# idonahum/photoVerse

Hardware: AMD Instinct MI355X
Metric: denoising steps/sec at 512x512 bs=16, 50-step loop (2 UNet fwd + CFG + DPM-Solver++ step per step) (higher is better)
Workload: dtype f16; 1 GPU; configs[1] shape timed over 96 steps instead of 50: SD-v1.5 UNet + PhotoVerse processors, 96-step loop, bs=16/GPU, 512x512 (64x64 latents), P=1, guidance 7.5, fp16; per_gpu_batch=16, global_batch=16, latent=64, parallelism=dp1 (batch-sharded, 1 all_gather), hip_graph=True, graph_branches=2

## Files before the change

### photoverse_amd/csrc/pv_attn.hip

```cpp
#include "pv_common.h"
#include <type_traits>

#ifndef PV_ATTN8_DEFAULT
#define PV_ATTN8_DEFAULT 497
#endif
#ifndef PV_ATTN8_FENCE_LOOP
#define PV_ATTN8_FENCE_LOOP 1
#endif
#ifndef PV_ATTN8_MAX3
#define PV_ATTN8_MAX3 1
#endif
#ifndef PV_ATTN8_RECOMPUTE
#define PV_ATTN8_RECOMPUTE 1
#endif
#ifndef PV_ATTN8_REDO_HINT
#define PV_ATTN8_REDO_HINT 0
#endif
#ifndef PV_ATTN8_LOOP_PAD
#define PV_ATTN8_LOOP_PAD 4
#endif
#ifndef PV_ATTN_LAZY_UP
#define PV_ATTN_LAZY_UP 8.f
#endif
#ifndef PV_ATTN_ABLATE
#define PV_ATTN_ABLATE 0
#endif

#ifdef PV_ATTN8_STAMPS
__device__ unsigned long long pv_attn8_stamps[3 * 8 * 8];
extern "C" int pv_attn8_read_stamps(unsigned long long* out) { return (int)hipMemcpyFromSymbol(out, HIP_SYMBOL(pv_attn8_stamps), sizeof(pv_attn8_stamps)); }
#define A8_NOW() __builtin_amdgcn_s_memtime()
#endif

namespace {

template <int D>
struct ACfg {
    static constexpr int DK = (D + 31) / 32 * 32;
    static constexpr int KSTEPS = DK / 32;
    static constexpr int DVF = (D + 15) / 16;
    static constexpr bool KSWZ = DK == 64;
    static constexpr int KS = KSWZ ? DK : DK + 8;
    static constexpr int KCH = KS / 8;
    __device__ static __forceinline__ int koff(int row, int chunk) {
        return KSWZ ? row * KS + ((chunk ^ (row & 7)) << 3) : row * KS + (chunk << 3);
    }
    static constexpr int vs_dwords() {
        int v = DVF * 8;
        while ((v & 63) != 8 && (v & 63) != 24 && (v & 63) != 40 && (v & 63) != 56) v += 4;
        return v;
    }
    static constexpr int VS = vs_dwords() * 2;
    static constexpr int CH = D / 8;
};

__device__ __forceinline__ half8_t zero8() { return half8_t{0, 0, 0, 0, 0, 0, 0, 0}; }

__device__ __forceinline__ half8_t vt_frag(const half_t* sV, int VS, int key0, int dv0, int fr, int fq) {
    const half_t* a = sV + (key0 + fq * 4 + (fr >> 2)) * VS + dv0 + (fr & 3) * 4;
    const fp16x4_t t1 = __builtin_amdgcn_ds_read_tr16_b64_v4f16((__attribute__((address_space(3))) fp16x4_t*)(a));
    const fp16x4_t t2 = __builtin_amdgcn_ds_read_tr16_b64_v4f16((__attribute__((address_space(3))) fp16x4_t*)(a + 16 * VS));
    half8_t r;
#pragma unroll
    for (int j = 0; j < 4; ++j) {
        r[j] = (half_t)t1[j];
        r[j + 4] = (half_t)t2[j];
    }
    return r;
}

template <int D>
constexpr int attn_min_waves() { return 1; }

template <int D, int NQ, bool DMA>
__global__ __launch_bounds__(256, attn_min_waves<D>()) void attn_kernel(const pv_attn_params p) {
    using C = ACfg<D>;
    static_assert(!DMA || (C::KSWZ && C::VS == 48 && D == 40), "the DMA staging is laid out for d = 40 (128-B swizzled K rows, 96-B V rows)");
    constexpr int KB = 64;
    constexpr int NCHUNK = KB * C::CH;
    constexpr int KPT = (NCHUNK + 255) / 256;
#ifdef PV_ATTN_NO_ONES
    constexpr bool ONES = false;
#else
    constexpr bool ONES = (D % 16) != 0;
#endif
    constexpr bool DBUF = false;
    constexpr int STAGE = KB * (C::KS + C::VS);
    extern __shared__ __attribute__((aligned(16))) char smem[];
    half_t* sbase = reinterpret_cast<half_t*>(smem);

    const int tid = threadIdx.x, lane = tid & 63, wave = pv_wave_id();
    const int fr = lane & 15, fq = lane >> 4;
    constexpr int QW = 64 * NQ;
    const int nqt = (p.nq + QW - 1) / QW;
    const int rid = pv_xcd_remap((int)blockIdx.x, (int)gridDim.x);
    const int qt = rid % nqt, h = (rid / nqt) % p.heads, b = rid / (nqt * p.heads);
    const half_t* Q = reinterpret_cast<const half_t*>(p.q) + (size_t)b * p.nq * p.ldq + h * D;
    const half_t* Kg = reinterpret_cast<const half_t*>(p.k) + (size_t)b * p.nk * p.ldk + h * D;
    const half_t* Vg = reinterpret_cast<const half_t*>(p.v) + (size_t)b * p.nk * p.ldv + h * D;

    for (int st = 0; st < (DMA ? 4 : DBUF ? 2 : 1); ++st) {
        half_t* sK = sbase + st * STAGE;
        half_t* sV = sK + KB * C::KS;
        constexpr int NPC = C::KCH - C::CH, NPV = (C::VS - D) / 8;
        for (int i = tid; i < KB * NPC; i += 256) {
            const int r = i / NPC, c = i - r * NPC;
            *reinterpret_cast<half8_t*>(sK + C::koff(r, C::CH + c)) = zero8();
        }
        for (int i = tid; i < KB * NPV; i += 256) {
            const int r = i / NPV, c = i - r * NPV;
            half8_t v = zero8();
            if (ONES && c == 0) v[0] = (half_t)1.0f;
            *reinterpret_cast<half8_t*>(sV + r * C::VS + D + c * 8) = v;
        }
    }

    const float qscale = rsqrtf((float)D) * 1.4426950408889634f;
    half8_t qf[NQ][C::KSTEPS];
    int qrow[NQ];
#pragma unroll
    for (int qi = 0; qi < NQ; ++qi) {
        qrow[qi] = qt * QW + (wave * NQ + qi) * 16 + fr;
        const int rc = min(qrow[qi], p.nq - 1);
#pragma unroll
        for (int ks = 0; ks < C::KSTEPS; ++ks) {
            const int c = ks * 4 + fq;
            qf[qi][ks] = c < C::CH ? *reinterpret_cast<const half8_t*>(Q + (size_t)rc * p.ldq + c * 8) : zero8();
#pragma unroll
            for (int j = 0; j < 8; ++j) qf[qi][ks][j] = (half_t)((float)qf[qi][ks][j] * qscale);
        }
    }

    half8_t kreg[KPT], vreg[KPT];
    auto gload = [&](int t) {
#pragma unroll
        for (int i = 0; i < KPT; ++i) {
            const int idx = tid + i * 256;
            const int key = idx / C::CH, c = idx - key * C::CH;
            const int gk = t * KB + key;
            if (idx < NCHUNK && gk < p.nk) {
                kreg[i] = *reinterpret_cast<const half8_t*>(Kg + (size_t)gk * p.ldk + c * 8);
                vreg[i] = *reinterpret_cast<const half8_t*>(Vg + (size_t)gk * p.ldv + c * 8);
            } else {
                kreg[i] = zero8();
                vreg[i] = zero8();
            }
        }
    };
    auto swrite = [&](int st) {
        half_t* sK = sbase + st * STAGE;
        half_t* sV = sK + KB * C::KS;
#pragma unroll
        for (int i = 0; i < KPT; ++i) {
            const int idx = tid + i * 256;
            const int key = idx / C::CH, c = idx - key * C::CH;
            if (idx < NCHUNK) {
                *reinterpret_cast<half8_t*>(sK + C::koff(key, c)) = kreg[i];
                *reinterpret_cast<half8_t*>(sV + key * C::VS + c * 8) = vreg[i];
            }
        }
    };

    float4_t o[C::DVF][NQ];
#pragma unroll
    for (int f = 0; f < C::DVF; ++f)
#pragma unroll
        for (int qi = 0; qi < NQ; ++qi) o[f][qi] = float4_t{0.f, 0.f, 0.f, 0.f};
    float m_run[NQ], l_run[NQ];
#pragma unroll
    for (int qi = 0; qi < NQ; ++qi) m_run[qi] = l_run[qi] = 0.f;

    auto tile = [&](int t, int st, const bool MASKED, const bool FIRST) {
        const half_t* sK = sbase + st * STAGE;
        const half_t* sV = sK + KB * C::KS;
        float4_t s[4][NQ];
#pragma unroll
        for (int qi = 0; qi < NQ; ++qi) {
            const float init = FIRST ? 0.f : -m_run[qi];
#pragma unroll
            for (int kb = 0; kb < 4; ++kb) s[kb][qi] = float4_t{init, init, init, init};
        }
#pragma unroll
        for (int ks = 0; ks < C::KSTEPS; ++ks)
#pragma unroll
            for (int kb = 0; kb < 4; ++kb) {
                const half8_t a = *reinterpret_cast<const half8_t*>(sK + C::koff(kb * 16 + fr, ks * 4 + fq));
#pragma unroll
#if PV_ATTN_ABLATE == 2
                asm volatile("" ::"v"(a));
#else
                for (int qi = 0; qi < NQ; ++qi) s[kb][qi] = __builtin_amdgcn_mfma_f32_16x16x32_f16(a, qf[qi][ks], s[kb][qi], 0, 0, 0);
#endif
            }
        half8_t pb[2][NQ];
#pragma unroll
        for (int qi = 0; qi < NQ; ++qi) {
            if (MASKED) {
#pragma unroll
                for (int kb = 0; kb < 4; ++kb)
#pragma unroll
                    for (int r = 0; r < 4; ++r) {
                        const int key = t * KB + kb * 16 + fq * 4 + r;
                        if (key >= p.nk || (p.causal && key > qrow[qi])) s[kb][qi][r] = -INFINITY;
                    }
            }
            float mx = -INFINITY;
#pragma unroll
            for (int kb = 0; kb < 4; ++kb)
#pragma unroll
                for (int r = 0; r < 4; ++r) mx = fmaxf(mx, s[kb][qi][r]);
            mx = pv_quad_max(mx);
            float d = 0.f;
            if (FIRST || __any(mx > PV_ATTN_LAZY_UP)) {
                d = FIRST ? (mx == -INFINITY ? 0.f : mx) : fmaxf(mx, 0.f);
                const float alpha = FIRST ? 0.f : PV_EXP2(-d);
                m_run[qi] += d;
                if (!ONES) l_run[qi] *= alpha;
#pragma unroll
                for (int f = 0; f < C::DVF; ++f) o[f][qi] *= alpha;
#pragma unroll
                for (int kb = 0; kb < 4; ++kb)
#pragma unroll
                    for (int r = 0; r < 4; ++r) s[kb][qi][r] -= d;
            }
            float rs = 0.f;
#pragma unroll
            for (int kb = 0; kb < 4; ++kb)
#pragma unroll
                for (int r = 0; r < 4; ++r) {
#if PV_ATTN_ABLATE == 1
                    const float e = s[kb][qi][r];
#else
                    const float e = PV_EXP2(s[kb][qi][r]);
#endif
                    if (!ONES) rs += e;
                    s[kb][qi][r] = e;
                }
            if (!ONES) l_run[qi] += rs;
#pragma unroll
            for (int s2 = 0; s2 < 2; ++s2)
#pragma unroll
                for (int r = 0; r < 4; ++r) {
                    pb[s2][qi][r] = (half_t)s[2 * s2][qi][r];
                    pb[s2][qi][r + 4] = (half_t)s[2 * s2 + 1][qi][r];
                }
        }
#pragma unroll
        for (int s2 = 0; s2 < 2; ++s2)
#pragma unroll
            for (int f = 0; f < C::DVF; ++f) {
                const half8_t a = vt_frag(sV, C::VS, s2 * 32, f * 16, fr, fq);
#if PV_ATTN_ABLATE == 3
                asm volatile("" ::"v"(a), "v"(pb[s2][0]), "v"(pb[s2][1]));
#else
#pragma unroll
                for (int qi = 0; qi < NQ; ++qi) o[f][qi] = __builtin_amdgcn_mfma_f32_16x16x32_f16(a, pb[s2][qi], o[f][qi], 0, 0, 0);
#endif
            }
    };

    int ntiles = (p.nk + KB - 1) / KB;
    if (p.causal) ntiles = min(ntiles, (min(qt * QW + QW - 1, p.nq - 1)) / KB + 1);
    if constexpr (DMA) {
        const __amdgpu_buffer_rsrc_t rk = __builtin_amdgcn_make_buffer_rsrc(const_cast<half_t*>(Kg), 0, ((p.nk - 1) * p.ldk + D) * 2, 0x00020000);
        const __amdgpu_buffer_rsrc_t rv = __builtin_amdgcn_make_buffer_rsrc(const_cast<half_t*>(Vg), 0, ((p.nk - 1) * p.ldv + D) * 2, 0x00020000);
        constexpr unsigned OOB = 0x80000000u;
        unsigned koff[2], voff[2];
        bool vlive[2];
#pragma unroll
        for (int i = 0; i < 2; ++i) {
            const int r = 8 * (wave + 4 * i) + (lane >> 3), c = (lane & 7) ^ (lane >> 3);
            koff[i] = c < C::CH ? (unsigned)(r * p.ldk * 2 + c * 16) : OOB;
            const int q = 64 * (wave + 4 * i) + lane, vr = q / 6, vc = q - vr * 6;
            voff[i] = (unsigned)(vr * p.ldv * 2 + vc * 16);
            vlive[i] = vc < C::CH;
        }
        auto issue_tile = [&](int t) {
            char* sK = reinterpret_cast<char*>(sbase + (t & 3) * STAGE);
            char* sV = sK + KB * C::KS * 2;
            const int sk = t * KB * p.ldk * 2, sv = t * KB * p.ldv * 2;
#pragma unroll
            for (int i = 0; i < 2; ++i) __builtin_amdgcn_raw_ptr_buffer_load_lds(rk, PV_LDS_PTR(sK + (wave + 4 * i) * 1024), 16, (int)koff[i], sk, 0, 0);
            if (vlive[0]) __builtin_amdgcn_raw_ptr_buffer_load_lds(rv, PV_LDS_PTR(sV + wave * 1024), 16, (int)voff[0], sv, 0, 0);
            if (wave < 2) {
                if (vlive[1]) __builtin_amdgcn_raw_ptr_buffer_load_lds(rv, PV_LDS_PTR(sV + (wave + 4) * 1024), 16, (int)voff[1], sv, 0, 0);
            }
        };
        __syncthreads();
        issue_tile(0);
        if (ntiles > 1) issue_tile(1);
        for (int t = 0; t < ntiles; ++t) {
            if ((t & 1) == 0) {
                asm volatile("s_waitcnt vmcnt(0)" ::: "memory");
                asm volatile("s_waitcnt lgkmcnt(0)" ::: "memory");
                __builtin_amdgcn_s_barrier();
                asm volatile("" ::: "memory");
                if (t + 2 < ntiles) issue_tile(t + 2);
                if (t + 3 < ntiles) issue_tile(t + 3);
            }
            const bool need_mask = p.causal || (t + 1) * KB > p.nk;
            tile(t, t & 3, need_mask, t == 0);
        }
    } else {
    gload(0);
    if (DBUF) {
        swrite(0);
        __syncthreads();
    }
    for (int t = 0; t < ntiles; ++t) {
        const int st = DBUF ? (t & 1) : 0;
        if (!DBUF) {
            __syncthreads();
            swrite(0);
            __syncthreads();
        }
        if (t + 1 < ntiles) gload(t + 1);
        const bool need_mask = p.causal || (t + 1) * KB > p.nk;
        tile(t, st, need_mask, t == 0);
        if (DBUF) {
            if (t + 1 < ntiles) swrite(st ^ 1);
            __syncthreads();
        }
    }
    }

    half_t* O = reinterpret_cast<half_t*>(p.out) + (size_t)b * p.nq * p.ldo + h * D;
#pragma unroll
    for (int qi = 0; qi < NQ; ++qi) {
        float l;
        if (ONES) {
            l = __shfl(o[D / 16][qi][D % 4], fr + 16 * ((D % 16) / 4), 64);
        } else {
            l = pv_quad_sum(l_run[qi]);
        }
        const float inv = 1.0f / l;
        if (p.lse != nullptr && fq == 0 && qrow[qi] < p.nq) p.lse[((size_t)b * p.heads + h) * p.nq + qrow[qi]] = m_run[qi] + __log2f(l);
        if (qrow[qi] < p.nq) {
#pragma unroll
            for (int f = 0; f < C::DVF; ++f) {
                const int dv = f * 16 + fq * 4;
                if (dv < D) {
                    half4_t ov;
#pragma unroll
                    for (int r = 0; r < 4; ++r) ov[r] = (half_t)(o[f][qi][r] * inv);
                    *reinterpret_cast<half4_t*>(O + (size_t)qrow[qi] * p.ldo + dv) = ov;
                }
            }
        }
    }
}

template <int VAR>
__global__ __launch_bounds__(512, 2) void attn8_kernel(const pv_attn_params p) {
    constexpr int D = 40, NQ = 4, KB = 64;
    using C = ACfg<D>;
    constexpr bool STAGGER = (VAR & 1) != 0, PRIO = (VAR & 2) != 0, PCHECK = (VAR & 32) != 0, JOINT = (VAR & 4) != 0 || PCHECK, LAZY = (VAR & 8) != 0 || PCHECK;
    constexpr bool SEGPRIO = (VAR & 16) != 0, PREF = (VAR & 64) != 0, K48 = (VAR & 128) != 0;
    constexpr bool DMA_IN_VEC = PREF && (VAR & 256) != 0;
    constexpr float UP = LAZY ? 8.f : 0.f;
    constexpr int STAGE = KB * (C::KS + C::VS);
    extern __shared__ __attribute__((aligned(16))) char smem[];
    half_t* sbase = reinterpret_cast<half_t*>(smem);

    const int tid = threadIdx.x, lane = tid & 63, wave = pv_wave_id();
    const int fr = lane & 15, fq = lane >> 4;
    const bool late = STAGGER && wave >= 4;
    constexpr int QW = 64 * NQ * 2;
    const int nqt = (p.nq + QW - 1) / QW;
    const int rid = pv_xcd_remap((int)blockIdx.x, (int)gridDim.x);
    const int qt = rid % nqt, h = (rid / nqt) % p.heads, b = rid / (nqt * p.heads);
    const half_t* Q = reinterpret_cast<const half_t*>(p.q) + (size_t)b * p.nq * p.ldq + h * D;
    const half_t* Kg = reinterpret_cast<const half_t*>(p.k) + (size_t)b * p.nk * p.ldk + h * D;
    const half_t* Vg = reinterpret_cast<const half_t*>(p.v) + (size_t)b * p.nk * p.ldv + h * D;

    for (int st = 0; st < 4; ++st) {
        half_t* sK = sbase + st * STAGE;
        half_t* sV = sK + KB * C::KS;
        constexpr int NPC = C::KCH - C::CH, NPV = (C::VS - D) / 8;
        for (int i = tid; i < KB * NPC; i += 512) {
            const int r = i / NPC, c = i - r * NPC;
            *reinterpret_cast<half8_t*>(sK + C::koff(r, C::CH + c)) = zero8();
        }
        for (int i = tid; i < KB * NPV; i += 512) {
            const int r = i / NPV, c = i - r * NPV;
// ... 499 lines not shown
                    *reinterpret_cast<half4_t*>(O + (size_t)qrow[qi] * p.ldo + dv) = ov;
                }
            }
        }
    }
    }
}

enum AttnKind { ATTN8 = 0, ATTN40_4_DMA, ATTN40_2_DMA, ATTN_4, ATTN_2 };
struct AttnChoice {
    AttnKind kind;
    int var8;
    long wgs;
};
#define PV_A8_VARIANTS(X) X(0) X(1) X(9) X(13) X(33) X(49) X(73) X(201) X(225) X(241) X(481) X(497)
constexpr bool attn8_variant_built(int v) {
#define PV_A8_TEST(V) if (v == V) return true;
    PV_A8_VARIANTS(PV_A8_TEST)
#undef PV_A8_TEST
    return false;
}
static_assert(attn8_variant_built(PV_ATTN8_DEFAULT), "the default variant must be an instantiated one");

template <int D>
AttnChoice choose_attn(const pv_attn_params& p) {
    static const int nq_env = getenv("PV_ATTN_NQ") ? atoi(getenv("PV_ATTN_NQ")) : 0;
    const long wg256 = (long)((p.nq + 255) / 256) * p.heads * p.batch, wg128 = (long)((p.nq + 127) / 128) * p.heads * p.batch;
    const bool four = D == 40 && (nq_env ? nq_env == 4 : wg256 >= 1024);
    if constexpr (D == 40) {
        static const bool no_dma = getenv("PV_ATTN_NO_DMA") != nullptr;
        if (!no_dma && (size_t)p.nk * (size_t)(p.ldk > p.ldv ? p.ldk : p.ldv) * 2 < (1ull << 31)) {
            const char* env8 = getenv("PV_ATTN8");
            const char* env8min = getenv("PV_ATTN8_MIN");
            const int var8 = env8 ? atoi(env8) : PV_ATTN8_DEFAULT;
            const long wg512 = (long)((p.nq + 511) / 512) * p.heads * p.batch;
            if (attn8_variant_built(var8) && !p.causal && wg512 >= (env8min ? atol(env8min) : 256)) return {ATTN8, var8, wg512};
            return four ? AttnChoice{ATTN40_4_DMA, 0, wg256} : AttnChoice{ATTN40_2_DMA, 0, wg128};
        }
    }
    return four ? AttnChoice{ATTN_4, 0, wg256} : AttnChoice{ATTN_2, 0, wg128};
}

template <int D>
int launch_attn(const pv_attn_params& p, hipStream_t s) {
    using C = ACfg<D>;
    constexpr int smem1 = 64 * (C::KS + C::VS) * 2;
    const AttnChoice ch = choose_attn<D>(p);
    if constexpr (D == 40) {
        constexpr int smem3 = 4 * smem1;
        if (ch.kind == ATTN8) {
            void (*kern)(const pv_attn_params) = nullptr;
            switch (ch.var8) {
#define PV_A8_CASE(V) case V: kern = attn8_kernel<V>; break;
                PV_A8_VARIANTS(PV_A8_CASE)
#undef PV_A8_CASE
                default: return (int)hipErrorInvalidValue;
            }
            static bool attr8_set[64][512] = {};
            int dev8 = 0;
            (void)hipGetDevice(&dev8);
            if (!attr8_set[dev8 & 63][ch.var8 & 511]) {
                const hipError_t e = hipFuncSetAttribute(reinterpret_cast<const void*>(kern), hipFuncAttributeMaxDynamicSharedMemorySize, smem3);
                if (e != hipSuccess) return (int)e;
                attr8_set[dev8 & 63][ch.var8 & 511] = true;
            }
            hipLaunchKernelGGL(kern, dim3((unsigned)ch.wgs), dim3(512), smem3, s, p);
            return PV_CHECK_LAUNCH();
        }
        if (ch.kind == ATTN40_4_DMA || ch.kind == ATTN40_2_DMA) {
            static bool attr_set_dev[64] = {};
            int dev_id = 0;
            (void)hipGetDevice(&dev_id);
            if (!attr_set_dev[dev_id & 63]) {
                hipError_t e = hipFuncSetAttribute(reinterpret_cast<const void*>(attn_kernel<40, 4, true>), hipFuncAttributeMaxDynamicSharedMemorySize, smem3);
                if (e == hipSuccess) e = hipFuncSetAttribute(reinterpret_cast<const void*>(attn_kernel<40, 2, true>), hipFuncAttributeMaxDynamicSharedMemorySize, smem3);
                if (e != hipSuccess) return (int)e;
                attr_set_dev[dev_id & 63] = true;
            }
            if (ch.kind == ATTN40_4_DMA) hipLaunchKernelGGL((attn_kernel<40, 4, true>), dim3((unsigned)ch.wgs), dim3(256), smem3, s, p);
            else hipLaunchKernelGGL((attn_kernel<40, 2, true>), dim3((unsigned)ch.wgs), dim3(256), smem3, s, p);
            return PV_CHECK_LAUNCH();
        }
    }
    if (ch.kind == ATTN_4) hipLaunchKernelGGL((attn_kernel<D, D == 40 ? 4 : 2, false>), dim3((unsigned)ch.wgs), dim3(256), smem1, s, p);
    else hipLaunchKernelGGL((attn_kernel<D, 2, false>), dim3((unsigned)ch.wgs), dim3(256), smem1, s, p);
    return PV_CHECK_LAUNCH();
}

template <int D>
int attn_info(const pv_attn_params& p, char* name, int name_len, int64_t* workgroups) {
    const AttnChoice ch = choose_attn<D>(p);
    int n;
    switch (ch.kind) {
        case ATTN8: n = snprintf(name, (size_t)name_len, "attn8_kernel<%d>", ch.var8); break;
        case ATTN40_4_DMA: n = snprintf(name, (size_t)name_len, "attn_kernel<40, 4, true>"); break;
        case ATTN40_2_DMA: n = snprintf(name, (size_t)name_len, "attn_kernel<40, 2, true>"); break;
        case ATTN_4: n = snprintf(name, (size_t)name_len, "attn_kernel<%d, 4, false>", D); break;
        default: n = snprintf(name, (size_t)name_len, "attn_kernel<%d, 2, false>", D); break;
    }
    if (n < 0 || n >= name_len) return (int)hipErrorInvalidValue;
    if (workgroups) *workgroups = ch.wgs;
    return 0;
}

template <int D>
int launch_xattn(const pv_xattn_params& p, hipStream_t s) {
    using C = ACfg<D>;
    constexpr int smem = XKEYS * (C::KS + C::VS) * 2;
    static bool attr_set_dev[64] = {};
    int dev_id = 0;
    (void)hipGetDevice(&dev_id);
    bool& attr_set = attr_set_dev[dev_id & 63];
    if (smem > 48 * 1024 && !attr_set) {
        hipError_t e = hipFuncSetAttribute(reinterpret_cast<const void*>(xattn_kernel<D, false>), hipFuncAttributeMaxDynamicSharedMemorySize, smem);
        if (e == hipSuccess) e = hipFuncSetAttribute(reinterpret_cast<const void*>(xattn_kernel<D, true>), hipFuncAttributeMaxDynamicSharedMemorySize, smem);
        if (e != hipSuccess) return (int)e;
        attr_set = true;
    }
    const int nqt = (p.nq + 127) / 128;
    const long wgs = (long)nqt * p.heads * p.batch;
    int qt_per_wg = (int)(wgs / 1024);
    qt_per_wg = qt_per_wg < 1 ? 1 : (qt_per_wg > 4 ? 4 : qt_per_wg);
    const int nqg = (nqt + qt_per_wg - 1) / qt_per_wg;
    if (qt_per_wg > 1) hipLaunchKernelGGL((xattn_kernel<D, true>), dim3(nqg * p.heads * p.batch), dim3(256), smem, s, p, qt_per_wg);
    else hipLaunchKernelGGL((xattn_kernel<D, false>), dim3(nqg * p.heads * p.batch), dim3(256), smem, s, p, 1);
    return PV_CHECK_LAUNCH();
}

}

extern "C" int pv_attention(const pv_attn_params* p, void* stream) {
    if (!p->q || !p->k || !p->v || !p->out || p->batch <= 0 || p->heads <= 0 || p->nq <= 0 || p->nk <= 0 || (p->ldq % 8) ||
        (p->ldk % 8) || (p->ldv % 8) || (p->ldo % 4))
        return (int)hipErrorInvalidValue;
    hipStream_t s = (hipStream_t)stream;
    switch (p->d) {
        case 40: return launch_attn<40>(*p, s);
        case 64: return launch_attn<64>(*p, s);
        case 80: return launch_attn<80>(*p, s);
        case 160: return launch_attn<160>(*p, s);
        default: return (int)hipErrorInvalidValue;
    }
}

extern "C" int pv_attention_kernel_info(const pv_attn_params* p, char* name, int32_t name_len, int64_t* workgroups) {
    if (!p || !name || name_len <= 0 || p->batch <= 0 || p->heads <= 0 || p->nq <= 0 || p->nk <= 0) return (int)hipErrorInvalidValue;
    switch (p->d) {
        case 40: return attn_info<40>(*p, name, name_len, workgroups);
        case 64: return attn_info<64>(*p, name, name_len, workgroups);
        case 80: return attn_info<80>(*p, name, name_len, workgroups);
        case 160: return attn_info<160>(*p, name, name_len, workgroups);
        default: return (int)hipErrorInvalidValue;
    }
}

extern "C" int pv_cross_attention(const pv_xattn_params* p, void* stream) {
    if (!p->q || !p->kt || !p->vt || !p->kip || !p->vip || !p->out || p->batch <= 0 || p->heads <= 0 || p->nq <= 0 || p->nt <= 0 ||
        p->nt > IP0 || p->nip <= 0 || p->nip > XKEYS - IP0 || (p->ldq % 8) || (p->ldkt % 8) || (p->ldvt % 8) || (p->ldkip % 8) ||
        (p->ldvip % 8) || (p->ldo % 4))
        return (int)hipErrorInvalidValue;
    hipStream_t s = (hipStream_t)stream;
    switch (p->d) {
        case 40: return launch_xattn<40>(*p, s);
        case 80: return launch_xattn<80>(*p, s);
        case 160: return launch_xattn<160>(*p, s);
        default: return (int)hipErrorInvalidValue;
// ... 3 lines not shown
```

### photoverse_amd/build.py

```python
from __future__ import annotations

import concurrent.futures as cf
import os
import shutil
import subprocess
import sys

HERE = os.path.dirname(os.path.abspath(__file__))
CSRC = os.path.join(HERE, "csrc")
LIBDIR = os.path.join(HERE, "lib")
LIB = os.path.join(LIBDIR, "libphotoverse_hip.so")
SOURCES = ["pv_gemm.hip", "pv_convbig.hip", "pv_norm.hip", "pv_attn.hip", "pv_misc.hip", "pv_xfused.hip", "pv_xq.hip", "pv_rowgemm.hip", "pv_backward.hip", "pv_train.hip", "pv_attnbwd.hip"]
FLAGS = ["--offload-arch=gfx950", "-O3", "-std=c++17", "-fPIC"]
EXTRA_FLAGS = {"pv_attn.hip": ["-mllvm", "-amdgpu-mfma-vgpr-form", "-fno-honor-nans"],
               "pv_xfused.hip": ["-mllvm", "-amdgpu-mfma-vgpr-form", "-fno-honor-nans",
                                 "-mllvm", "-pragma-unroll-threshold=4000000"],

               "pv_xq.hip": ["-mllvm", "-amdgpu-mfma-vgpr-form", "-fno-honor-nans"],
               "pv_rowgemm.hip": ["-mllvm", "-amdgpu-mfma-vgpr-form"],
               "pv_train.hip": ["-mllvm", "-amdgpu-mfma-vgpr-form", "-fno-honor-nans"],
               "pv_attnbwd.hip": ["-mllvm", "-amdgpu-mfma-vgpr-form", "-fno-honor-nans"]}


def _hipcc() -> str:
    exe = shutil.which("hipcc") or "/opt/rocm/bin/hipcc"
    if not os.path.exists(exe):
        raise RuntimeError("hipcc not found: the HIP extension cannot be built")
    return exe


def _stale(out: str, deps) -> bool:
    if not os.path.exists(out):
        return True
    t = os.path.getmtime(out)
    return any(os.path.getmtime(d) > t for d in deps)


def build_lib(force: bool = False, verbose: bool = True) -> str:
    os.makedirs(LIBDIR, exist_ok=True)
    hipcc = _hipcc()
    headers = [os.path.join(CSRC, "pv_common.h"), os.path.join(CSRC, "pv_gemm_dev.h"), os.path.join(os.path.dirname(HERE), "include", "photoverse_hip.h"), __file__]
    objs, jobs = [], []
    for src in SOURCES:
        s = os.path.join(CSRC, src)
        o = os.path.join(LIBDIR, src.replace(".hip", ".o"))
        objs.append(o)
        if force or _stale(o, [s] + headers):
            jobs.append([hipcc, *FLAGS, *EXTRA_FLAGS.get(src, []), "-c", s, "-o", o])
    if jobs:
        with cf.ThreadPoolExecutor(max_workers=4) as ex:
            for cmd, res in zip(jobs, ex.map(lambda c: subprocess.run(c, capture_output=True, text=True), jobs)):
                if res.returncode != 0:
                    raise RuntimeError("hipcc failed: %s\n%s" % (" ".join(cmd), res.stderr))
                if verbose:
                    print("[photoverse_amd.build] compiled", os.path.basename(cmd[-3]))
    if jobs or force or _stale(LIB, objs):
        res = subprocess.run([hipcc, "--offload-arch=gfx950", "-shared", "-fPIC", "-o", LIB, *objs], capture_output=True, text=True)
        if res.returncode != 0:
            raise RuntimeError("link failed:\n" + res.stderr)
        if verbose:
            print("[photoverse_amd.build] linked", LIB)
    return LIB


if __name__ == "__main__":
    build_lib(force="--force" in sys.argv)
```

### photoverse_amd/csrc/pv_gemm.hip

```cpp
#include "pv_gemm_dev.h"

namespace {

constexpr int BK = 64;
constexpr int ROW_BYTES = BK * 2;

template <int NF, int MIV = 4>
struct TileCfg {
    static constexpr int MI = MIV;
    static constexpr int BM = 2 * MI * 16;
    static constexpr int BN = NF * 32;
    static constexpr int NWAVES = 4;
    static constexpr int THREADS = NWAVES * 64;
    static constexpr int A_PER_WAVE = BM / 8 / NWAVES;
    static constexpr int STAGES = 2;
    static constexpr int A_BYTES = BM * ROW_BYTES;
    static constexpr int B_BYTES = BN * ROW_BYTES;
    static constexpr int STAGE_BYTES = A_BYTES + B_BYTES;
    static constexpr int SMEM_BYTES = STAGES * STAGE_BYTES;
    static constexpr int B_PIECES = NF * 4;
    static constexpr int B_PER_WAVE = (B_PIECES + NWAVES - 1) / NWAVES;
};

__device__ __forceinline__ float epi_act(float x, int act) {
// ... 452 lines not shown

template <int NF>
int choose_tpw(const pv_gemm_params_dev& p) {
    static const int tpw_env = getenv("PV_GEMM_TPW") ? atoi(getenv("PV_GEMM_TPW")) : 0;
    if (p.taps != 1 || (p.splitk > 1 && p.splitk_ws)) return 1;
    const int tiles_n = p.N / (NF * 32), nk = (p.c0 + p.c1) / BK;
    const long nblk = (long)((p.M + 127) / 128) * tiles_n;
    if (tpw_env > 0) return tiles_n % tpw_env == 0 ? tpw_env : 1;
    for (int c = 8; c >= 2; --c)
        if (tiles_n % c == 0 && nk <= 5 && nblk / c >= 1024) return c;
    return 1;
}

template <int NF, bool CONV, bool GEGLU>
int dispatch(const pv_gemm_params_dev& p, hipStream_t stream) {
    if constexpr (!CONV && GEGLU) {
        const int tpw = choose_tpw<NF>(p);
        if (tpw > 1) return launch<NF, false, true, false, true>(p, stream, tpw);
    }
    if constexpr (!GEGLU) {
        if (p.colstats && !(p.splitk > 1 && p.splitk_ws)) return launch<NF, CONV, false, true>(p, stream);
    }
    if constexpr (!CONV && !GEGLU) {
        static const int mi2_env = getenv("PV_GEMM_MI2") ? atoi(getenv("PV_GEMM_MI2")) : 512;
        const long tiles128 = (long)((p.M + 127) / 128) * (p.N / (NF * 32));
        if (!(p.splitk > 1 && p.splitk_ws) && tiles128 < mi2_env) return launch<NF, false, false, false, false, 2>(p, stream);
    }
    return launch<NF, CONV, GEGLU>(p, stream);
}

}

int pv_gemm_splitk_reduce_launch(const pv_gemm_params_dev& p, int splits, hipStream_t stream) {
    hipLaunchKernelGGL(splitk_reduce_kernel, dim3((unsigned)((p.N + 63) / 64), (unsigned)((p.M + 63) / 64)), dim3(256), 0, stream, p, splits);
    return PV_CHECK_LAUNCH();
}

thread_local pv_launch_probe* pv_gemm_probe = nullptr;

extern "C" int pv_gemm_conv(const pv_gemm_params* pp, void* stream_);

extern "C" int pv_gemm_conv_kernel_info(const pv_gemm_params* pp, char* name, int32_t name_len, int64_t* workgroups) {
    if (!pp || !name || name_len <= 0) return (int)hipErrorInvalidValue;
    pv_launch_probe probe;
    probe.name[0] = 0;
    probe.wgs = 0;
    pv_gemm_probe = &probe;
    const int rc = pv_gemm_conv(pp, nullptr);
    pv_gemm_probe = nullptr;
    if (rc != 0) return rc;
    if ((int)strlen(probe.name) >= name_len) return (int)hipErrorInvalidValue;
    strcpy(name, probe.name);
    if (workgroups) *workgroups = probe.wgs;
    return 0;
}

extern "C" int pv_gemm_conv(const pv_gemm_params* pp, void* stream_) {
    pv_gemm_params_dev p;
    static_cast<pv_gemm_params&>(p) = *pp;
    hipStream_t stream = reinterpret_cast<hipStream_t>(stream_);
    const int cin = p.c0 + p.c1;
    if (p.M <= 0 || p.N <= 0 || cin <= 0 || (cin % 64) || (p.c0 % 64) || (p.taps != 1 && p.taps != 9) || p.act == PV_ACT_GELU || p.splitk < 0 || p.splitk > 16 ||
        !p.a0 || !p.w || !p.out || (p.c1 && !p.a1) || p.hout * p.wout <= 0)
        return (int)hipErrorInvalidValue;
    if (p.colstats && (p.geglu || p.out_f32)) return (int)hipErrorInvalidValue;
    if (p.taps == 9 && !(p.pad == 1 || (p.pad == 0 && p.stride == 2 && !p.upsample))) return (int)hipErrorInvalidValue;
    {
        const size_t a_rows = p.taps == 9 ? (size_t)p.batch * p.hin * p.win : (size_t)p.M;
        const size_t b0 = ((a_rows - 1) * p.lda0 + p.c0) * 2, b1 = p.c1 ? ((a_rows - 1) * p.lda1 + p.c1) * 2 : 0;
        const size_t bw = (size_t)p.N * p.taps * cin * 2;
        if (b0 >= (1ull << 31) || b1 >= (1ull << 31) || bw >= (1ull << 31)) return (int)hipErrorInvalidValue;
        p.a0_bytes = (uint32_t)b0;
        p.a1_bytes = (uint32_t)b1;
        p.w_bytes = (uint32_t)bw;
    }
    if (p.geglu && (p.taps != 1 || (p.N % 128))) return (int)hipErrorInvalidValue;
    if (p.a_norm && (p.taps != 9 || (p.a_norm_act != PV_ACT_NONE && p.a_norm_act != PV_ACT_SILU))) return (int)hipErrorInvalidValue;
    {
        const int rc = pv_conv_big_launch(p, stream);
        if (rc >= 0) return rc;
        if (rc == -2 || p.a_norm) return (int)hipErrorInvalidValue;
    }
    if (p.ln_rowsum) return (int)hipErrorInvalidValue;
    if (p.geglu) return dispatch<4, false, true>(p, stream);
    const bool conv = p.taps == 9;
    if (p.N % 160 == 0) return conv ? dispatch<5, true, false>(p, stream) : dispatch<5, false, false>(p, stream);
    if (p.N % 128 == 0) return conv ? dispatch<4, true, false>(p, stream) : dispatch<4, false, false>(p, stream);
    return (int)hipErrorInvalidValue;
}
```

### photoverse_amd/csrc/pv_gemm_dev.h

```cpp
#pragma once
#include "pv_common.h"

struct pv_gemm_params_dev : pv_gemm_params {
    uint32_t a0_bytes, a1_bytes, w_bytes;
};

__attribute__((visibility("hidden"))) int pv_conv_big_launch(const pv_gemm_params_dev& p, hipStream_t stream);


__attribute__((visibility("hidden"))) int pv_gemm_splitk_reduce_launch(const pv_gemm_params_dev& p, int splits, hipStream_t stream);


struct pv_launch_probe {
    char name[160];
    long wgs;
};
extern thread_local pv_launch_probe* pv_gemm_probe;
```

Baseline: 33.21 denoising steps/s (bs=16 per GPU, summed over GPUs).

## Add DMA ring-buffer K/V staging for d=80 and d=160 attention

For head dims 80 and 160, the attention kernel now stages K/V tiles through a multi-slot LDS ring filled by buffer_load_lds DMA, replacing the register gload/swrite path with its two barriers per tile. It uses an unpadded row layout with XOR swizzles and handles the 16-wide tail of d=80 through a zero-padded 32-wide MFMA. The aim is to overlap global loads with compute and drop the register round trip and the padding. In exchange it uses more LDS, which may lower occupancy, and keeps a synchronous fallback for offsets too large for a buffer descriptor.

```diff
diff --git a/photoverse_amd/csrc/pv_attn.hip b/photoverse_amd/csrc/pv_attn.hip
--- a/photoverse_amd/csrc/pv_attn.hip
+++ b/photoverse_amd/csrc/pv_attn.hip
@@ -52,7 +52,36 @@
     }
     static constexpr int VS = vs_dwords() * 2;
     static constexpr int CH = D / 8;
+    static constexpr bool TAIL16 = false;
+    __device__ static __forceinline__ int vchunk(int, int chunk) { return chunk; }
+    __device__ static __forceinline__ int vcol(int f, int) { return f * 16; }
 };
+
+template <int D>
+struct RCfg {
+    static_assert(D == 80 || D == 160, "row layouts worked out for 160-B and 320-B rows");
+    static constexpr int DK = D;
+    static constexpr int KSTEPS = D / 32;
+    static constexpr bool TAIL16 = (D % 32) == 16;
+    static constexpr int DVF = D / 16;
+    static constexpr bool KSWZ = D == 160;
+    static constexpr int KS = D, KCH = D / 8, VS = D, CH = D / 8;
+    __device__ static __forceinline__ int kchunk(int row, int chunk) { return KSWZ ? chunk ^ ((0 - (row >> 2)) & 3) : chunk; }
+    __device__ static __forceinline__ int koff(int row, int chunk) { return row * KS + (kchunk(row, chunk) << 3); }
+    __device__ static __forceinline__ int vchunk(int row, int chunk) { return KSWZ ? chunk ^ (((row >> 2) & 1) << 1) : chunk; }
+    __device__ static __forceinline__ int vcol(int f, int fq) { return (KSWZ ? f ^ (fq & 1) : f) * 16; }
+};
+#ifndef PV_ATTN_RING_SLOTS80
+#define PV_ATTN_RING_SLOTS80 2
+#endif
+#ifndef PV_ATTN_RING_SLOTS160
+#define PV_ATTN_RING_SLOTS160 2
+#endif
+#ifndef PV_ATTN_RING_TAIL32
+#define PV_ATTN_RING_TAIL32 1
+#endif
+template <int D, bool DMA>
+constexpr int attn_ring_slots() { return DMA ? 0 : D == 80 ? PV_ATTN_RING_SLOTS80 : D == 160 ? PV_ATTN_RING_SLOTS160 : 0; }
 
 __device__ __forceinline__ half8_t zero8() { return half8_t{0, 0, 0, 0, 0, 0, 0, 0}; }
 
@@ -74,8 +103,11 @@
 
 template <int D, int NQ, bool DMA>
 __global__ __launch_bounds__(256, attn_min_waves<D>()) void attn_kernel(const pv_attn_params p) {
-    using C = ACfg<D>;
-    static_assert(!DMA || (C::KSWZ && C::VS == 48 && D == 40), "the DMA staging is laid out for d = 40 (128-B swizzled K rows, 96-B V rows)");
+    constexpr int NS = attn_ring_slots<D, DMA>();
+    constexpr bool RING = NS != 0;
+    using C = std::conditional_t<RING, RCfg<D>, ACfg<D>>;
+    static_assert(!DMA || (C::KSWZ && C::VS == 48 && D == 40), "the d = 40 DMA staging is laid out for 128-B swizzled K rows and 96-B V rows");
+    static_assert(!RING || (NQ == 2 && (NS == 2 || NS == 4)), "ring form: <80 / 160, 2, false> with two or four slots");
     constexpr int KB = 64;
     constexpr int NCHUNK = KB * C::CH;
     constexpr int KPT = (NCHUNK + 255) / 256;
@@ -99,7 +131,7 @@
     const half_t* Kg = reinterpret_cast<const half_t*>(p.k) + (size_t)b * p.nk * p.ldk + h * D;
     const half_t* Vg = reinterpret_cast<const half_t*>(p.v) + (size_t)b * p.nk * p.ldv + h * D;
 
-    for (int st = 0; st < (DMA ? 4 : DBUF ? 2 : 1); ++st) {
+    for (int st = 0; st < (RING ? 0 : DMA ? 4 : DBUF ? 2 : 1); ++st) {
         half_t* sK = sbase + st * STAGE;
         half_t* sV = sK + KB * C::KS;
         constexpr int NPC = C::KCH - C::CH, NPV = (C::VS - D) / 8;
@@ -128,6 +160,15 @@
             qf[qi][ks] = c < C::CH ? *reinterpret_cast<const half8_t*>(Q + (size_t)rc * p.ldq + c * 8) : zero8();
 #pragma unroll
             for (int j = 0; j < 8; ++j) qf[qi][ks][j] = (half_t)((float)qf[qi][ks][j] * qscale);
+        }
+    }
+    half4_t qf4[NQ];
+    if constexpr (C::TAIL16) {
+#pragma unroll
+        for (int qi = 0; qi < NQ; ++qi) {
+            qf4[qi] = *reinterpret_cast<const half4_t*>(Q + (size_t)min(qrow[qi], p.nq - 1) * p.ldq + C::KSTEPS * 32 + fq * 4);
+#pragma unroll
+            for (int j = 0; j < 4; ++j) qf4[qi][j] = (half_t)((float)qf4[qi][j] * qscale);
         }
     }
 
@@ -156,7 +197,7 @@
             const int key = idx / C::CH, c = idx - key * C::CH;
             if (idx < NCHUNK) {
                 *reinterpret_cast<half8_t*>(sK + C::koff(key, c)) = kreg[i];
-                *reinterpret_cast<half8_t*>(sV + key * C::VS + c * 8) = vreg[i];
+                *reinterpret_cast<half8_t*>(sV + key * C::VS + C::vchunk(key, c) * 8) = vreg[i];
             }
         }
     };
@@ -192,6 +233,24 @@
                 for (int qi = 0; qi < NQ; ++qi) s[kb][qi] = __builtin_amdgcn_mfma_f32_16x16x32_f16(a, qf[qi][ks], s[kb][qi], 0, 0, 0);
 #endif
             }
+        if constexpr (C::TAIL16) {
+            if (!PV_ATTN_RING_TAIL32) __builtin_amdgcn_sched_barrier(0);
+#pragma unroll
+            for (int kb = 0; kb < 4; ++kb) {
+                const half4_t a = *reinterpret_cast<const half4_t*>(sK + C::koff(kb * 16 + fr, C::KSTEPS * 4 + (fq >> 1)) + (fq & 1) * 4);
+#if PV_ATTN_ABLATE == 2
+                asm volatile("" ::"v"(a));
+#elif PV_ATTN_RING_TAIL32
+                const half8_t a8{a[0], a[1], a[2], a[3], 0, 0, 0, 0};
+#pragma unroll
+                for (int qi = 0; qi < NQ; ++qi)
+                    s[kb][qi] = __builtin_amdgcn_mfma_f32_16x16x32_f16(a8, half8_t{qf4[qi][0], qf4[qi][1], qf4[qi][2], qf4[qi][3], 0, 0, 0, 0}, s[kb][qi], 0, 0, 0);
+#else
+#pragma unroll
+                for (int qi = 0; qi < NQ; ++qi) s[kb][qi] = __builtin_amdgcn_mfma_f32_16x16x16f16(a, qf4[qi], s[kb][qi], 0, 0, 0);
+#endif
+            }
+        }
         half8_t pb[2][NQ];
 #pragma unroll
         for (int qi = 0; qi < NQ; ++qi) {
@@ -249,7 +308,7 @@
         for (int s2 = 0; s2 < 2; ++s2)
 #pragma unroll
             for (int f = 0; f < C::DVF; ++f) {
-                const half8_t a = vt_frag(sV, C::VS, s2 * 32, f * 16, fr, fq);
+                const half8_t a = vt_frag(sV, C::VS, s2 * 32, C::vcol(f, fq), fr, fq);
 #if PV_ATTN_ABLATE == 3
                 asm volatile("" ::"v"(a), "v"(pb[s2][0]), "v"(pb[s2][1]));
 #else
@@ -300,6 +359,57 @@
             }
             const bool need_mask = p.causal || (t + 1) * KB > p.nk;
             tile(t, t & 3, need_mask, t == 0);
+        }
+    } else if constexpr (RING) {
+        constexpr int ROWB = D * 2, TILEB = KB * ROWB, NKP = TILEB / 1024, PPW = 2 * NKP / 4, G = NS / 2;
+        static_assert(TILEB % 1024 == 0 && (2 * NKP) % 4 == 0 && STAGE * 2 == 2 * TILEB, "a slot is a whole number of pieces per wave");
+        const size_t ldmax = (size_t)(p.ldk > p.ldv ? p.ldk : p.ldv);
+        if (((size_t)p.nk + KB) * ldmax * 2 < (1ull << 31)) {
+            const __amdgpu_buffer_rsrc_t rk = __builtin_amdgcn_make_buffer_rsrc(const_cast<half_t*>(Kg), 0, ((p.nk - 1) * p.ldk + D) * 2, 0x00020000);
+            const __amdgpu_buffer_rsrc_t rv = __builtin_amdgcn_make_buffer_rsrc(const_cast<half_t*>(Vg), 0, ((p.nk - 1) * p.ldv + D) * 2, 0x00020000);
+            unsigned off[PPW];
+#pragma unroll
+            for (int i = 0; i < PPW; ++i) {
+                const int j = wave + 4 * i;
+                const bool isv = j >= NKP;
+                const int pos = (isv ? j - NKP : j) * 1024 + lane * 16, r = pos / ROWB, pc = (pos - r * ROWB) >> 4;
+                off[i] = (unsigned)(r * (isv ? p.ldv : p.ldk) * 2 + (isv ? C::vchunk(r, pc) : C::kchunk(r, pc)) * 16);
+            }
+            auto issue_tile = [&](int t) {
+                char* slot = reinterpret_cast<char*>(sbase + (t % NS) * STAGE);
+                const int sk = t * KB * p.ldk * 2, sv = t * KB * p.ldv * 2;
+#pragma unroll
+                for (int i = 0; i < PPW; ++i) {
+                    const int j = wave + 4 * i;
+                    if (j < NKP) __builtin_amdgcn_raw_ptr_buffer_load_lds(rk, PV_LDS_PTR(slot + j * 1024), 16, (int)off[i], sk, 0, 0);
+                    else __builtin_amdgcn_raw_ptr_buffer_load_lds(rv, PV_LDS_PTR(slot + j * 1024), 16, (int)off[i], sv, 0, 0);
+                }
+            };
+#pragma unroll
+            for (int i = 0; i < G; ++i)
+                if (i < ntiles) issue_tile(i);
+            for (int t = 0; t < ntiles; ++t) {
+                if (t % G == 0) {
+                    asm volatile("s_waitcnt vmcnt(0)" ::: "memory");
+                    asm volatile("s_waitcnt lgkmcnt(0)" ::: "memory");
+                    __builtin_amdgcn_s_barrier();
+                    asm volatile("" ::: "memory");
+#pragma unroll
+                    for (int i = 0; i < G; ++i)
+                        if (t + G + i < ntiles) issue_tile(t + G + i);
+                }
+                const bool need_mask = p.causal || (t + 1) * KB > p.nk;
+                tile(t, t % NS, need_mask, t == 0);
+            }
+        } else {
+            for (int t = 0; t < ntiles; ++t) {
+                gload(t);
+                __syncthreads();
+                swrite(0);
+                __syncthreads();
+                const bool need_mask = p.causal || (t + 1) * KB > p.nk;
+                tile(t, 0, need_mask, t == 0);
+            }
         }
     } else {
     gload(0);
@@ -965,6 +1075,22 @@
             return PV_CHECK_LAUNCH();
         }
     }
+    if constexpr (attn_ring_slots<D, false>() != 0) {
+        constexpr int smem_ring = attn_ring_slots<D, false>() * 64 * (RCfg<D>::KS + RCfg<D>::VS) * 2;
+        static_assert(smem_ring <= 160 * 1024, "the ring must fit a CU's LDS");
+        if constexpr (smem_ring > 48 * 1024) {
+            static bool attr_set_dev[64] = {};
+            int dev_id = 0;
+            (void)hipGetDevice(&dev_id);
+            if (!attr_set_dev[dev_id & 63]) {
+                const hipError_t e = hipFuncSetAttribute(reinterpret_cast<const void*>(attn_kernel<D, 2, false>), hipFuncAttributeMaxDynamicSharedMemorySize, smem_ring);
+                if (e != hipSuccess) return (int)e;
+                attr_set_dev[dev_id & 63] = true;
+            }
+        }
+        hipLaunchKernelGGL((attn_kernel<D, 2, false>), dim3((unsigned)ch.wgs), dim3(256), smem_ring, s, p);
+        return PV_CHECK_LAUNCH();
+    }
     if (ch.kind == ATTN_4) hipLaunchKernelGGL((attn_kernel<D, D == 40 ? 4 : 2, false>), dim3((unsigned)ch.wgs), dim3(256), smem1, s, p);
     else hipLaunchKernelGGL((attn_kernel<D, 2, false>), dim3((unsigned)ch.wgs), dim3(256), smem1, s, p);
     return PV_CHECK_LAUNCH();
```

Result: no change. 33.39 denoising steps/s (bs=16 per GPU, summed over GPUs), median of 6 (+0.6%).

## Add weight-stationary persistent kernel for 320x320 linear layers with residual

Applied to the files above, without the earlier changes.

Adds a persistent GEMM kernel for 1x1 linears with K=N=320 and large M. Each workgroup keeps the whole 320x320 weight in registers and streams 64-row A tiles through a 2- or 4-slot LDS ring using buffer-load-to-LDS DMA. The epilogue fuses bias, residual and optional column statistics. By default the path only takes residual-bearing linears, which targets the attention output projections at the highest-resolution UNet level and avoids reloading weight tiles. The trade-offs are high register pressure (launch_bounds 256,1), a grid capped at the CU count, and env-var gating for the other cases.

```diff
diff --git a/photoverse_amd/build.py b/photoverse_amd/build.py
--- a/photoverse_amd/build.py
+++ b/photoverse_amd/build.py
@@ -10,7 +10,7 @@
 CSRC = os.path.join(HERE, "csrc")
 LIBDIR = os.path.join(HERE, "lib")
 LIB = os.path.join(LIBDIR, "libphotoverse_hip.so")
-SOURCES = ["pv_gemm.hip", "pv_convbig.hip", "pv_norm.hip", "pv_attn.hip", "pv_misc.hip", "pv_xfused.hip", "pv_xq.hip", "pv_rowgemm.hip", "pv_backward.hip", "pv_train.hip", "pv_attnbwd.hip"]
+SOURCES = ["pv_gemm.hip", "pv_linws.hip", "pv_convbig.hip", "pv_norm.hip", "pv_attn.hip", "pv_misc.hip", "pv_xfused.hip", "pv_xq.hip", "pv_rowgemm.hip", "pv_backward.hip", "pv_train.hip", "pv_attnbwd.hip"]
 FLAGS = ["--offload-arch=gfx950", "-O3", "-std=c++17", "-fPIC"]
 EXTRA_FLAGS = {"pv_attn.hip": ["-mllvm", "-amdgpu-mfma-vgpr-form", "-fno-honor-nans"],
                "pv_xfused.hip": ["-mllvm", "-amdgpu-mfma-vgpr-form", "-fno-honor-nans",
diff --git a/photoverse_amd/csrc/pv_gemm.hip b/photoverse_amd/csrc/pv_gemm.hip
--- a/photoverse_amd/csrc/pv_gemm.hip
+++ b/photoverse_amd/csrc/pv_gemm.hip
@@ -558,6 +558,10 @@
         if (rc == -2 || p.a_norm) return (int)hipErrorInvalidValue;
     }
     if (p.ln_rowsum) return (int)hipErrorInvalidValue;
+    {
+        const int rc = pv_linear_ws_launch(p, stream);
+        if (rc >= 0) return rc;
+    }
     if (p.geglu) return dispatch<4, false, true>(p, stream);
     const bool conv = p.taps == 9;
     if (p.N % 160 == 0) return conv ? dispatch<5, true, false>(p, stream) : dispatch<5, false, false>(p, stream);
diff --git a/photoverse_amd/csrc/pv_gemm_dev.h b/photoverse_amd/csrc/pv_gemm_dev.h
--- a/photoverse_amd/csrc/pv_gemm_dev.h
+++ b/photoverse_amd/csrc/pv_gemm_dev.h
@@ -7,6 +7,9 @@
 
 __attribute__((visibility("hidden"))) int pv_conv_big_launch(const pv_gemm_params_dev& p, hipStream_t stream);
 
+#define PV_LINEAR_WS_MIN_DEFAULT 65536L
+#define PV_LINEAR_WS_SLOTS_DEFAULT 4
+__attribute__((visibility("hidden"))) int pv_linear_ws_launch(const pv_gemm_params_dev& p, hipStream_t stream);
 
 __attribute__((visibility("hidden"))) int pv_gemm_splitk_reduce_launch(const pv_gemm_params_dev& p, int splits, hipStream_t stream);
 
diff --git a/photoverse_amd/csrc/pv_linws.hip b/photoverse_amd/csrc/pv_linws.hip
--- /dev/null
+++ b/photoverse_amd/csrc/pv_linws.hip
@@ -0,0 +1,256 @@
+#include "pv_gemm_dev.h"
+#include <stdlib.h>
+
+namespace {
+
+constexpr int WS_C = 320;
+constexpr int WS_BM = 64;
+constexpr int WS_NF = 5, WS_MI = 4, WS_KK = WS_C / 32;
+constexpr int WS_SUB = WS_BM * 128;
+constexpr int WS_SLOT = WS_BM * WS_C * 2;
+constexpr int WS_DMA = WS_SLOT / 1024 / 4;
+constexpr int WS_RLOADS = WS_NF * WS_MI;
+
+template <int N>
+__device__ __forceinline__ void ws_wait_vmcnt() {
+    static_assert(N >= 0 && N < 64, "vmcnt is a 6-bit field");
+    asm volatile("s_waitcnt vmcnt(%0)" ::"n"(N) : "memory");
+}
+
+template <int EXTRA>
+__device__ __forceinline__ void ws_wait_block(int blocks) {
+    if (blocks >= 3) ws_wait_vmcnt<3 * WS_DMA + EXTRA>();
+    else if (blocks == 2) ws_wait_vmcnt<2 * WS_DMA + EXTRA>();
+    else if (blocks == 1) ws_wait_vmcnt<WS_DMA + EXTRA>();
+    else ws_wait_vmcnt<EXTRA>();
+}
+
+__device__ __forceinline__ float ws_row16_sum(float v) {
+    v += __builtin_bit_cast(float, __builtin_amdgcn_update_dpp(0, __builtin_bit_cast(int, v), 0x128, 0xf, 0xf, false));
+    v += __builtin_bit_cast(float, __builtin_amdgcn_update_dpp(0, __builtin_bit_cast(int, v), 0x124, 0xf, 0xf, false));
+    v += __builtin_bit_cast(float, __builtin_amdgcn_update_dpp(0, __builtin_bit_cast(int, v), 0x122, 0xf, 0xf, false));
+    v += __builtin_bit_cast(float, __builtin_amdgcn_update_dpp(0, __builtin_bit_cast(int, v), 0x121, 0xf, 0xf, false));
+    return v;
+}
+
+__device__ __forceinline__ half8_t ws_frag(const char* sub, int row, int chunk) {
+    return *reinterpret_cast<const half8_t*>(sub + row * 128 + ((chunk ^ (row & 7)) << 4));
+}
+
+template <bool CS, bool RES, int SLOTS>
+__global__ __launch_bounds__(256, 1) void linear_ws_kernel(const pv_gemm_params_dev p, const int nblocks) {
+    static_assert(SLOTS == 2 || SLOTS == 4, "ring of two or four 40-KB slots");
+    constexpr int NF = WS_NF, MI = WS_MI, KK = WS_KK;
+    extern __shared__ __attribute__((aligned(16))) char smem[];
+
+    const int lane = pv_lane_id(), wave = pv_wave_id();
+    const int fr = lane & 15, fq = lane >> 4;
+    const int grid = (int)gridDim.x, bid = (int)blockIdx.x;
+    const int nb = (nblocks - bid + grid - 1) / grid;
+
+    half8_t wf[NF][KK];
+    {
+        const half_t* wp = reinterpret_cast<const half_t*>(p.w) + (size_t)(wave * (NF * 16) + fr) * WS_C + fq * 8;
+#pragma unroll
+        for (int ni = 0; ni < NF; ++ni)
+#pragma unroll
+            for (int kk = 0; kk < KK; ++kk) wf[ni][kk] = *reinterpret_cast<const half8_t*>(wp + ni * 16 * WS_C + kk * 32);
+    }
+    const int nbase = wave * (NF * 16) + fq * 4;
+    float4_t bias_v[NF];
+#pragma unroll
+    for (int ni = 0; ni < NF; ++ni)
+        bias_v[ni] = p.bias ? *reinterpret_cast<const float4_t*>(p.bias + nbase + ni * 16) : float4_t{0.f, 0.f, 0.f, 0.f};
+    __builtin_amdgcn_sched_barrier(0);
+
+    const int lrow = lane >> 3;
+    const int lane_cc2 = ((lane & 7) ^ lrow) * 16;
+    constexpr unsigned OOB = 0x80000000u;
+    const __amdgpu_buffer_rsrc_t ra0 = __builtin_amdgcn_make_buffer_rsrc(const_cast<void*>(p.a0), 0, (int)p.a0_bytes, 0x00020000);
+    auto issue = [&](int i) {
+        const int m0 = (bid + i * grid) * WS_BM;
+        char* slot = smem + (i & (SLOTS - 1)) * WS_SLOT;
+        unsigned base[2];
+#pragma unroll
+        for (int h = 0; h < 2; ++h) {
+            const int m = m0 + (wave + 4 * h) * 8 + lrow;
+            base[h] = m < p.M ? (unsigned)m * (unsigned)(p.lda0 * 2) + lane_cc2 : OOB;
+        }
+#pragma unroll
+        for (int j = 0; j < WS_DMA; ++j) {
+            const int kc = j >> 1;
+            __builtin_amdgcn_raw_ptr_buffer_load_lds(ra0, PV_LDS_PTR(slot + (wave + 4 * j) * 1024), 16, (int)(base[j & 1] + (unsigned)(kc * 128)), 0, 0, 0);
+        }
+    };
+#pragma unroll
+    for (int s = 0; s < SLOTS; ++s) issue(s);
+
+    const bool want_cs = CS && p.colstats != nullptr;
+
+    ws_wait_vmcnt<(SLOTS - 1) * WS_DMA>();
+    __builtin_amdgcn_s_barrier();
+    asm volatile("" ::: "memory");
+
+    for (int i = 0; i < nb; ++i) {
+        const int m0 = (bid + i * grid) * WS_BM;
+        const char* slot = smem + (i & (SLOTS - 1)) * WS_SLOT;
+
+        half4_t res[NF][MI];
+        if (RES) {
+#pragma unroll
+            for (int mi = 0; mi < MI; ++mi) {
+                const int m = min(m0 + mi * 16 + fr, p.M - 1);
+#pragma unroll
+                for (int ni = 0; ni < NF; ++ni)
+                    res[ni][mi] = *reinterpret_cast<const half4_t*>(reinterpret_cast<const half_t*>(p.residual) + (size_t)m * p.ldr + nbase + ni * 16);
+            }
+        }
+
+        float4_t acc[NF][MI];
+#pragma unroll
+        for (int ni = 0; ni < NF; ++ni)
+#pragma unroll
+            for (int mi = 0; mi < MI; ++mi) acc[ni][mi] = float4_t{0.f, 0.f, 0.f, 0.f};
+
+        half8_t xa[2][MI];
+#pragma unroll
+        for (int mi = 0; mi < MI; ++mi) xa[0][mi] = ws_frag(slot, mi * 16 + fr, fq);
+#pragma unroll
+        for (int kk = 0; kk < KK; ++kk) {
+            if (kk + 1 < KK) {
+#pragma unroll
+                for (int mi = 0; mi < MI; ++mi)
+                    xa[(kk + 1) & 1][mi] = ws_frag(slot + ((kk + 1) >> 1) * WS_SUB, mi * 16 + fr, ((kk + 1) & 1) * 4 + fq);
+            }
+            __builtin_amdgcn_sched_barrier(0);
+#pragma unroll
+            for (int ni = 0; ni < NF; ++ni)
+#pragma unroll
+                for (int mi = 0; mi < MI; ++mi)
+                    acc[ni][mi] = __builtin_amdgcn_mfma_f32_16x16x32_f16(wf[ni][kk], xa[kk & 1][mi], acc[ni][mi], 0, 0, 0);
+            __builtin_amdgcn_sched_barrier(0);
+        }
+
+        if (i + 1 < nb) {
+            asm volatile("s_waitcnt lgkmcnt(0)" ::: "memory");
+            ws_wait_block<RES ? WS_RLOADS : 0>(min(SLOTS - 2, nb - 2 - i));
+            __builtin_amdgcn_s_barrier();
+            asm volatile("" ::: "memory");
+        }
+
+        float4_t cs[NF], cq[NF];
+#pragma unroll
+        for (int ni = 0; ni < NF; ++ni) cs[ni] = cq[ni] = float4_t{0.f, 0.f, 0.f, 0.f};
+#pragma unroll
+        for (int mi = 0; mi < MI; ++mi) {
+            const int m = m0 + mi * 16 + fr;
+            if (m >= p.M) continue;
+            unsigned pk[NF][2];
+#pragma unroll
+            for (int ni = 0; ni < NF; ++ni) {
+                float4_t v = acc[ni][mi] + bias_v[ni];
+                if (RES) {
+#pragma unroll
+                    for (int r = 0; r < 4; ++r) v[r] += (float)res[ni][mi][r];
+                }
+                const half4_t hv = half4_t{(half_t)v[0], (half_t)v[1], (half_t)v[2], (half_t)v[3]};
+                pk[ni][0] = __builtin_bit_cast(unsigned, half2_t{hv[0], hv[1]});
+                pk[ni][1] = __builtin_bit_cast(unsigned, half2_t{hv[2], hv[3]});
+                if (want_cs) {
+#pragma unroll
+                    for (int r = 0; r < 4; ++r) {
+                        const float f = (float)hv[r];
+                        cs[ni][r] += f;
+                        cq[ni][r] += f * f;
+                    }
+                }
+            }
+            half_t* orow = reinterpret_cast<half_t*>(p.out) + (size_t)m * p.ldc + wave * (NF * 16);
+            typedef unsigned uint4_t __attribute__((ext_vector_type(4)));
+            typedef unsigned uint2_t __attribute__((ext_vector_type(2)));
+#pragma unroll
+            for (int q = 0; q < NF / 2; ++q) {
+                const auto r0 = __builtin_amdgcn_permlane16_swap(pk[2 * q][0], pk[2 * q + 1][0], false, false);
+                const auto r1 = __builtin_amdgcn_permlane16_swap(pk[2 * q][1], pk[2 * q + 1][1], false, false);
+                const unsigned a0 = r0[0], b0 = r0[1], a1 = r1[0], b1 = r1[1];
+                const int col = (fq & 1) ? (2 * q + 1) * 16 + (fq - 1) * 4 : (2 * q) * 16 + fq * 4;
+                *reinterpret_cast<uint4_t*>(orow + col) = uint4_t{a0, a1, b0, b1};
+            }
+            *reinterpret_cast<uint2_t*>(orow + (NF - 1) * 16 + fq * 4) = uint2_t{pk[NF - 1][0], pk[NF - 1][1]};
+        }
+        if (want_cs) {
+#pragma unroll
+            for (int ni = 0; ni < NF; ++ni)
+#pragma unroll
+                for (int r = 0; r < 4; ++r) {
+                    cs[ni][r] = ws_row16_sum(cs[ni][r]);
+                    cq[ni][r] = ws_row16_sum(cq[ni][r]);
+                }
+            if (fr == 0) {
+                float* dst = p.colstats + ((size_t)(m0 / 64) * 2) * p.N + nbase;
+#pragma unroll
+                for (int ni = 0; ni < NF; ++ni) {
+                    *reinterpret_cast<float4_t*>(dst + ni * 16) = cs[ni];
+                    *reinterpret_cast<float4_t*>(dst + p.N + ni * 16) = cq[ni];
+                }
+            }
+        }
+
+        if (i + SLOTS < nb) issue(i + SLOTS);
+    }
+}
+
+int ws_cus() {
+    static int cus_dev[64] = {};
+    int dev_id = 0;
+    if (hipGetDevice(&dev_id) != hipSuccess) return 256;
+    int& cus = cus_dev[dev_id & 63];
+    if (cus <= 0) {
+        int v = 0;
+        cus = (hipDeviceGetAttribute(&v, hipDeviceAttributeMultiprocessorCount, dev_id) == hipSuccess && v > 0) ? v : 256;
+    }
+    return cus;
+}
+
+template <bool CS, bool RES, int SLOTS>
+int launch_ws(const pv_gemm_params_dev& p, hipStream_t stream) {
+    const int nblocks = (p.M + WS_BM - 1) / WS_BM;
+    const int grid = min(ws_cus(), nblocks);
+    if (pv_gemm_probe) {
+        snprintf(pv_gemm_probe->name, sizeof(pv_gemm_probe->name), "linear_ws_kernel<%s, %s, %d>", CS ? "true" : "false", RES ? "true" : "false", SLOTS);
+        pv_gemm_probe->wgs = grid;
+        return 0;
+    }
+    static bool attr_set_dev[64] = {};
+    int dev_id = 0;
+    (void)hipGetDevice(&dev_id);
+    bool& attr_set = attr_set_dev[dev_id & 63];
+    auto kern = linear_ws_kernel<CS, RES, SLOTS>;
+    if (!attr_set) {
+        hipError_t e = hipFuncSetAttribute(reinterpret_cast<const void*>(kern), hipFuncAttributeMaxDynamicSharedMemorySize, SLOTS * WS_SLOT);
+        if (e != hipSuccess) return (int)e;
+        attr_set = true;
+    }
+    hipLaunchKernelGGL(kern, dim3(grid), dim3(256), SLOTS * WS_SLOT, stream, p, nblocks);
+    return PV_CHECK_LAUNCH();
+}
+
+template <int SLOTS>
+int dispatch_ws(const pv_gemm_params_dev& p, hipStream_t stream) {
+    if (p.colstats) return p.residual ? launch_ws<true, true, SLOTS>(p, stream) : launch_ws<true, false, SLOTS>(p, stream);
+    return p.residual ? launch_ws<false, true, SLOTS>(p, stream) : launch_ws<false, false, SLOTS>(p, stream);
+}
+
+}
+
+int pv_linear_ws_launch(const pv_gemm_params_dev& p, hipStream_t stream) {
+    const char* env = getenv("PV_LINEAR_WS_MIN");
+    const long ws_min = env ? atol(env) : PV_LINEAR_WS_MIN_DEFAULT;
+    if (!env && !p.residual) return -1;
+    if (p.taps != 1 || p.c0 != WS_C || p.c1 != 0 || p.N != WS_C || p.geglu || p.out_f32 || p.act != PV_ACT_NONE || p.rowadd || p.ln_rowsum || p.a_norm ||
+        (p.splitk > 1 && p.splitk_ws) || ws_min <= 0 || p.M < ws_min)
+        return -1;
+    const char* senv = getenv("PV_LINEAR_WS_SLOTS");
+    const int slots = senv ? atoi(senv) : PV_LINEAR_WS_SLOTS_DEFAULT;
+    return slots == 2 ? dispatch_ws<2>(p, stream) : dispatch_ws<4>(p, stream);
+}
```

New measurement: 33.62 denoising steps/s (bs=16 per GPU, summed over GPUs) before, 33.83 denoising steps/s (bs=16 per GPU, summed over GPUs) after (median of 6 runs). About the same (+0.6%).
